# Christina-hshi/SH-assembly

Hardware: AMD Instinct MI355X
Metric: k-mers counted/sec (whole node), CQF build, C.elegans-like k=47 (higher is better)
Workload: dtype u64

## Files before the change

### sh-assembly_amd/csrc/cqf_kernels.hip

```cpp
#include "shk_device.h"

#define SHK_EMPTY 0xFFFFFFFFu
#define SHK_SUM_STRIDE 8
#define SHK_CNT_NOVER 4
#define SHK_CNT_ISLOTS 5
#define SHK_NCOUNTERS 6
#define SHK_SPILL_LENS SHK_REGION
#define SHK_SPILL_STRIDE 768
#define SHK_NC_CAP 128
#define SHK_SPILL_PACK_MAX (SHK_SPILL_STRIDE - SHK_SPILL_LENS)
#define SHK_RSCAN_TILE 4096

struct ShkMergeArgs {
  const uint8_t *tabA;
  uint8_t *tabB;
  const uint64_t *finA;
  uint64_t *finB;
  const uint32_t *words;
  const uint64_t *region_base;
  uint32_t region_cap;
  uint64_t nslots, xnslots, nblocks;
  uint64_t q_lo;
  uint32_t hb;
  uint32_t chunk_lo, chunk_hi;
  int want_hist;
  int denoise;
  uint32_t *summary;
  unsigned long long *counters;
  uint32_t *err;
  unsigned long long *dbg;
  uint32_t ablate;
  uint8_t *spill;
  const uint8_t *orec;
  uint32_t *over_list;
  unsigned long long *n_over;
  const uint32_t *list;
  uint16_t *newchunks;
  unsigned long long *chist;
  uint32_t split;
  uint32_t *isum;
  uint8_t *ilens;
  const uint64_t *prot_list;
  uint32_t nprot;
  uint32_t r0;
  uint32_t rstride;
  int counted;
};

__device__ __forceinline__ unsigned shk_img_slot_off(unsigned p) {
  return (p >> 6) * SHK_BLOCK_BYTES + SHK_OFF_SLOTS + (p & 63);
}

__device__ __forceinline__ unsigned shk_img_dec(const uint8_t *img, unsigned pos, unsigned run_end, unsigned *rem_out,
                                                uint64_t *count) {
  unsigned rem = img[shk_img_slot_off(pos)];
  *rem_out = rem;
  if (pos == run_end) { *count = 1; return 1; }
  unsigned digit = img[shk_img_slot_off(pos + 1)];
  if (digit > rem) { *count = 1; return 1; }
  unsigned n = 1;
  uint64_t cnt = 0;
  if (digit == 0) { n++; digit = img[shk_img_slot_off(pos + n)]; }
  while ((digit & 0x80) && pos + n < run_end) { cnt = cnt * 128 + (digit & 0x7f); n++; digit = img[shk_img_slot_off(pos + n)]; }
  cnt = cnt * 128 + (digit & 0x7f);
  *count = cnt + 1;
  return n + 1;
}

__device__ __forceinline__ ShkMP shk_block_exscan_mp(ShkMP v, ShkMP *total, long long *sa, long long *sb) {
  const unsigned lane = shk_lane(), wave = shk_wave(), nw = blockDim.x / SHK_WAVE;
  ShkMP incl = v;
  for (int d = 1; d < SHK_WAVE; d <<= 1) {
    ShkMP y;
    y.a = __shfl_up(incl.a, d);
    y.b = __shfl_up(incl.b, d);
    if (lane >= (unsigned)d) incl = shk_mp_compose(y, incl);
  }
  if (lane == SHK_WAVE - 1) { sa[wave] = incl.a; sb[wave] = incl.b; }
  __syncthreads();
  if (threadIdx.x == 0) {
    ShkMP run; run.a = 0; run.b = SHK_NEG_INF;
    for (unsigned w = 0; w < nw; w++) {
      ShkMP cur; cur.a = sa[w]; cur.b = sb[w];
      sa[w] = run.a; sb[w] = run.b;
      run = shk_mp_compose(run, cur);
    }
    sa[SHK_MAX_WAVES] = run.a; sb[SHK_MAX_WAVES] = run.b;
  }
  __syncthreads();
  ShkMP pre; pre.a = sa[wave]; pre.b = sb[wave];
  ShkMP prev;
  prev.a = __shfl_up(incl.a, 1);
  prev.b = __shfl_up(incl.b, 1);
  if (lane == 0) { prev.a = 0; prev.b = SHK_NEG_INF; }
  ShkMP res = shk_mp_compose(pre, prev);
  total->a = sa[SHK_MAX_WAVES];
  total->b = sb[SHK_MAX_WAVES];
  __syncthreads();
  return res;
}

__device__ __forceinline__ unsigned shk_enc_len_fast(unsigned rem, uint64_t total) {
  if (total <= 1) return (unsigned)total;
  if (total <= 128) return 2u + ((unsigned)(total - 1) > rem ? 1u : 0u);
  return shk_enc_len(rem, total);
}
__device__ __forceinline__ unsigned shk_img_dec_fast(const uint8_t *img, unsigned pos, unsigned run_end, unsigned *rem_out,
                                                     uint64_t *count) {
  const unsigned rem = img[shk_img_slot_off(pos)];
  *rem_out = rem;
  if (pos == run_end) { *count = 1; return 1; }
  const unsigned d = img[shk_img_slot_off(pos + 1)];
  if (d > rem) { *count = 1; return 1; }
  if (d != 0 && d < 0x80) { *count = (uint64_t)d + 1; return 2; }
  return shk_img_dec(img, pos, run_end, rem_out, count);
}

__device__ __forceinline__ unsigned shk_flat_dec(const uint8_t *s, unsigned pos, unsigned run_end, unsigned *rem_out, uint64_t *count) {
  unsigned rem = s[pos];
  *rem_out = rem;
  if (pos == run_end) { *count = 1; return 1; }
  unsigned digit = s[pos + 1];
  if (digit > rem) { *count = 1; return 1; }
  unsigned n = 1;
  uint64_t cnt = 0;
  if (digit == 0) { n++; digit = s[pos + n]; }
  while ((digit & 0x80) && pos + n < run_end) { cnt = cnt * 128 + (digit & 0x7f); n++; digit = s[pos + n]; }
  cnt = cnt * 128 + (digit & 0x7f);
  *count = cnt + 1;
  return n + 1;
}
__device__ __forceinline__ unsigned shk_flat_dec_fast(const uint8_t *s, unsigned pos, unsigned run_end, unsigned *rem_out, uint64_t *count) {
  const unsigned rem = s[pos];
  *rem_out = rem;
  if (pos == run_end) { *count = 1; return 1; }
  const unsigned d = s[pos + 1];
  if (d > rem) { *count = 1; return 1; }
  if (d != 0 && d < 0x80) { *count = (uint64_t)d + 1; return 2; }
  return shk_flat_dec(s, pos, run_end, rem_out, count);
}

template <int IMGB>
__device__ __forceinline__ void shk_store_image(const ShkMergeArgs &A, uint32_t r, uint32_t nregions, const uint8_t *nimg,
                                                unsigned tid, uint32_t nown, uint64_t b0, uint64_t q0, uint32_t out_lo,
                                                uint32_t out_hi, bool new_any, long long fout_rel) {
  if (r == nregions - 1) {
    const long long fend = fout_rel + (long long)q0;
    for (uint64_t b = A.nslots / 64 + tid; b < A.nblocks; b += SHK_WAVE) {
      long long o = fend - (long long)(64 * b);
      A.tabB[b * SHK_BLOCK_BYTES] = (uint8_t)(o < 0 ? 0 : (o > 255 ? 255 : o));
    }
  }

  uint8_t *tb = A.tabB + b0 * SHK_BLOCK_BYTES;
  uint32_t vblk = nown;
  if (new_any && out_lo == 0 && (nown * SHK_BLOCK_BYTES) % 4 == 0) {
    vblk = 0;
    const uint32_t *src = reinterpret_cast<const uint32_t *>(nimg);
    uint32_t *dst = reinterpret_cast<uint32_t *>(tb);
    for (uint32_t i = tid; i < nown * SHK_BLOCK_BYTES / 4; i += SHK_WAVE) dst[i] = src[i];
  }
  for (uint32_t i = tid; i < vblk * 9; i += SHK_WAVE) {
    const uint32_t blk = i / 9, byte = i % 9;
    tb[blk * SHK_BLOCK_BYTES + byte] = nimg[blk * SHK_BLOCK_BYTES + byte];
  }
  if (out_hi > out_lo) {
    const uint32_t va = vblk * 64, vb = nown * 64;
    for (uint32_t p = out_lo + tid; p < out_hi; p += SHK_WAVE)
      if (p < va || p >= vb || vblk == nown) tb[shk_img_slot_off(p)] = nimg[shk_img_slot_off(p)];
    const uint32_t m0 = out_lo >> 3, m1 = (out_hi - 1) >> 3;
    for (uint32_t m = m0 + tid; m <= m1; m += SHK_WAVE) {
      const uint32_t bo = (m >> 3) * SHK_BLOCK_BYTES + SHK_OFF_RUN + (m & 7);
      const uint8_t v = nimg[bo];
      if (vblk < nown && (m >> 3) >= vblk && (m >> 3) < nown) continue;
      if (m == m0 || m == m1) {
        if (v) {
          uint8_t *addr = tb + bo;
          uintptr_t ai = reinterpret_cast<uintptr_t>(addr);
          uint32_t *w = reinterpret_cast<uint32_t *>(ai & ~(uintptr_t)3);
          atomicOr(w, (uint32_t)v << ((ai & 3) << 3));
        }
      } else {
        tb[bo] = v;
      }
    }
  }
}

#define SHK_STAGE_PER_LANE 32
#define SHK_STAGE_STRIDE 36

#define SHK_STAMP(i) do { if (A.dbg && (blockIdx.x & 63) == 0 && threadIdx.x == 0) { unsigned long long t_ = __builtin_amdgcn_s_memtime(); atomicAdd(&A.dbg[i], t_ - t_prev); t_prev = t_; } } while (0)

template <int MODE, int IMGB, bool FUSED = false, bool OLDREC = false>
__global__ void __launch_bounds__(SHK_MERGE_GROUP) k_region_merge(ShkMergeArgs A) {
  static_assert(!FUSED || MODE == 3, "the one-pass deNoise point is a spill-mode pass");
  static_assert(!OLDREC || MODE == 0 || MODE == 3, "the write pass reads the table");
  constexpr bool WRITE = MODE == 1;
  constexpr bool STAGE = WRITE || MODE == 3;
  constexpr unsigned IMG_BLOCKS = IMGB, IMG_SLOTS = IMGB * 64, IMG_BYTES = IMGB * SHK_BLOCK_BYTES;
  static_assert(IMGB <= SHK_WAVE, "one lane per image block in the rank/select step");
  __shared__ __attribute__((aligned(16))) uint32_t hkey[SHK_HCAP];
  __shared__ __attribute__((aligned(16))) uint32_t hcnt[SHK_HCAP];
  __shared__ uint32_t s_added_b;
  __shared__ __attribute__((aligned(16))) uint16_t qcnt[SHK_REGION];
  uint32_t *qcntw = reinterpret_cast<uint32_t *>(qcnt);
  __shared__ uint16_t qoff[SHK_REGION + 2];
  __shared__ uint16_t nidx[SHK_HCAP];
  __shared__ __attribute__((aligned(8))) uint16_t orend[SHK_REGION];
  __shared__ uint16_t rstart[SHK_REGION];
  __shared__ __attribute__((aligned(16))) uint8_t oimg[IMG_BYTES + 16];
  __shared__ __attribute__((aligned(16))) uint8_t nimg[IMG_BYTES + 16];
  __shared__ __attribute__((aligned(16))) uint8_t opk[SHK_SPILL_PACK_MAX + 16];
  __shared__ __attribute__((aligned(16))) uint8_t stage[SHK_MERGE_THREADS * SHK_STAGE_STRIDE];
  __shared__ uint64_t oocc[SHK_REGION_BLOCKS];
  __shared__ uint64_t orunw[IMG_BLOCKS];
  __shared__ uint32_t oorank[SHK_REGION_BLOCKS + 1];
  __shared__ uint32_t orrank[IMG_BLOCKS + 1];
  __shared__ uint32_t s_fail, s_added, s_nlist;
  uint32_t *hidle = reinterpret_cast<uint32_t *>(orend);

  unsigned long long t_prev = A.dbg ? __builtin_amdgcn_s_memtime() : 0;
  const unsigned tid = threadIdx.x;
  const unsigned ngrp = blockDim.x;
  constexpr unsigned nthr = SHK_MERGE_THREADS;
  const uint32_t r = A.list ? A.list[blockIdx.x] : (blockIdx.x + A.r0) * A.rstride;
  const uint32_t nregions = (uint32_t)((A.nslots + SHK_REGION - 1) / SHK_REGION);
  const uint64_t q0 = (uint64_t)r * SHK_REGION;
  const uint32_t nq = (uint32_t)((A.nslots - q0) < SHK_REGION ? (A.nslots - q0) : SHK_REGION);
  const uint32_t nown = (nq + 63) / 64;
  const uint64_t b0 = q0 / 64;

  const uint64_t fa0 = A.finA[r], fa1 = A.finA[r + 1];
  const uint64_t olo_abs = fa0 > q0 ? fa0 : q0;
  const bool old_any = fa1 > olo_abs;
  const uint32_t olo = (uint32_t)(olo_abs - q0);
  const uint32_t ohi = old_any ? (uint32_t)((fa1 - q0) > 0xFFFFFFF ? 0xFFFFFFF : (fa1 - q0)) : olo;
  uint32_t nblk_old = old_any ? (ohi + 63) / 64 : 0;
  if (nblk_old < nown) nblk_old = nown;
  if (tid == 0) { s_fail = 0; s_added = 0; s_nlist = 0; s_added_b = 0; }
  uint16_t *slist = reinterpret_cast<uint16_t *>(stage);
  bool fatal = false;
  if (!OLDREC && (nblk_old > IMG_BLOCKS || ohi > IMG_SLOTS)) {
    if (tid == 0) atomicOr(A.err, SHK_E_OLD_EXTENT);
    fatal = true;
    nblk_old = nown;
  }
  if (b0 + nblk_old > A.nblocks) nblk_old = (uint32_t)(A.nblocks - b0);

  if ((MODE == 0 || MODE == 3) && !old_any && !fatal && (!A.words || (A.region_cap ? A.region_base[r] == (uint64_t)r * A.region_cap : A.region_base[r] == A.region_base[r + 1]))) {
    if (tid < SHK_SUM_STRIDE) A.summary[(size_t)SHK_SUM_STRIDE * r + tid] = 0;
    if (MODE == 3 && tid < SHK_WAVE) reinterpret_cast<uint32_t *>(A.spill + (size_t)r * SHK_SPILL_STRIDE)[tid] = 0;
    if (FUSED) {
      if (tid < 2) A.isum[2 * (size_t)r + tid] = 0;
      if (tid < SHK_WAVE) reinterpret_cast<uint32_t *>(A.ilens + (size_t)r * SHK_REGION)[tid] = 0;
    }
    return;
  }

  uint32_t ol4 = 0, oex = 0;
  bool orec_bad = false;
  {
    if (OLDREC) {
      if (tid < SHK_WAVE) {
        const uint32_t *src = reinterpret_cast<const uint32_t *>(A.orec + (size_t)r * SHK_SPILL_STRIDE);
        ol4 = src[tid];
        const uint32_t mine = (ol4 & 255u) + ((ol4 >> 8) & 255u) + ((ol4 >> 16) & 255u) + (ol4 >> 24);
        const uint32_t sincl = shk_wave_incl_add(mine);
        oex = sincl - mine;
        uint32_t ototal = (uint32_t)__builtin_amdgcn_readlane((int)sincl, SHK_WAVE - 1);
        if (ototal > SHK_SPILL_PACK_MAX) { orec_bad = true; ototal = 0; ol4 = 0; }
        uint32_t *dst = reinterpret_cast<uint32_t *>(opk);
        for (uint32_t i = tid; i < (ototal + 3) / 4; i += SHK_WAVE) dst[i] = src[SHK_SPILL_LENS / 4 + i];
      }
    } else {
    const uint32_t nbytes = nblk_old * SHK_BLOCK_BYTES;
    const uint32_t *src = reinterpret_cast<const uint32_t *>(A.tabA + b0 * SHK_BLOCK_BYTES);
    uint32_t *dst = reinterpret_cast<uint32_t *>(oimg);
    if (!(A.ablate & 64)) for (uint32_t i = tid; i < (nbytes + 3) / 4; i += ngrp) dst[i] = src[i];
    }
    {
      const uint4 e4 = make_uint4(SHK_EMPTY, SHK_EMPTY, SHK_EMPTY, SHK_EMPTY), z4 = make_uint4(0, 0, 0, 0);
      for (uint32_t i = tid; i < SHK_HCAP / 4; i += ngrp) reinterpret_cast<uint4 *>(hkey)[i] = e4;
      for (uint32_t i = tid; i < SHK_HCAP / 4; i += ngrp) reinterpret_cast<uint4 *>(hcnt)[i] = z4;
      for (uint32_t i = tid; i < SHK_REGION / 8; i += ngrp) reinterpret_cast<uint4 *>(qcnt)[i] = z4;
    }
    if (tid < 2 * SHK_WAVE) hidle[tid] = 0;
    if (WRITE) {
      uint32_t *z = reinterpret_cast<uint32_t *>(nimg);
      for (uint32_t i = tid; i < (IMG_BYTES + 16) / 4; i += ngrp) z[i] = 0;
    }
  }
  __syncthreads();

  SHK_STAMP(0);
  uint32_t my_added = 0, my_added_b = 0;
  if (A.words && !fatal && !(A.ablate & 1)) {
    const uint64_t kb = A.region_cap ? (uint64_t)r * A.region_cap : A.region_base[r], ke = A.region_cap ? A.region_base[r] : A.region_base[r + 1];
    const unsigned lane = shk_lane();
    const bool wh = A.want_hist != 0;
    bool corrupt = false, hfull = false;
    const uint32_t nw = (uint32_t)(ke - kb);
    if (FUSED && ((ke - kb) >= 32768 || A.counted) && tid == 0) atomicOr(A.err, SHK_E_FUSED);
    const uint32_t *wp = A.words + kb;
    for (uint32_t i0 = 0; i0 < nw; i0 += 4 * ngrp) {
      uint32_t wv[4];
#pragma unroll
      for (int u = 0; u < 4; u++) {
        const uint32_t i = i0 + (uint32_t)u * ngrp + tid;
        wv[u] = i < nw ? wp[i] : ~0u;
      }
      uint32_t h[4], want[4], chk[4], wgt[4];
      bool pend[4], bef[4];
#pragma unroll
      for (int u = 0; u < 4; u++) {
        const uint32_t w = wv[u];
        const bool in = i0 + (uint32_t)u * ngrp + tid < nw;
        const uint32_t chunk = w & (SHK_MAX_CHUNKS - 1);
        const uint32_t tag = (w >> SHK_CHUNK_BITS) & 0xFFFFu;
        const bool inr = in && (A.counted || (chunk >= A.chunk_lo && chunk <= A.chunk_hi));
        corrupt |= inr && (tag >> 8) >= nq;
        pend[u] = inr && (tag >> 8) < nq;
        want[u] = tag << SHK_CHUNK_BITS;
        chk[u] = chunk;
        wgt[u] = A.counted ? chunk + 1u : 1u;
        bef[u] = FUSED && chunk <= A.split;
        h[u] = (__umul24(tag, 40503u) & 0xFFFFu) >> (16 - SHK_HCAP_LOG2);
        my_added += (pend[u] && !bef[u]) ? wgt[u] : 0u;
        if (FUSED) my_added_b += (pend[u] && bef[u]) ? wgt[u] : 0u;
      }
      if (A.ablate & 256) continue;
      uint32_t guard = 0;
      while (__ballot(pend[0] || pend[1] || pend[2] || pend[3])) {
#pragma unroll
        for (int u = 0; u < 4; u++) {
          if (!__ballot(pend[u])) continue;
          const uint32_t prev = atomicCAS(pend[u] ? &hkey[h[u]] : &hidle[lane], pend[u] ? SHK_EMPTY : 0xFFFFFFFEu, want[u] | (SHK_MAX_CHUNKS - 1));
          const bool ins = pend[u] && prev == SHK_EMPTY;
          const uint32_t now = ins ? want[u] : prev;
          const bool match = pend[u] && (now >> SHK_CHUNK_BITS) == (want[u] >> SHK_CHUNK_BITS);
          const unsigned long long mi = __ballot(ins);
          if (mi) {
            const unsigned first = (unsigned)(__ffsll((long long)mi) - 1);
            uint32_t base = 0;
            if (lane == first) base = atomicAdd(&s_nlist, (uint32_t)__popcll(mi));
            base = (uint32_t)__builtin_amdgcn_readlane((int)base, (int)first);
            if (ins) slist[base + (uint32_t)__popcll(mi & ((1ULL << lane) - 1))] = (uint16_t)h[u];
          }
          if (wh) atomicMin(match ? &hkey[h[u]] : &hidle[lane], match ? (want[u] | chk[u]) : 0xFFFFFFFFu);
          atomicAdd(match ? &hcnt[h[u]] : &hidle[lane], match ? ((FUSED && !bef[u]) ? wgt[u] << 16 : wgt[u]) : 0u);
          pend[u] = pend[u] && !match;
          h[u] = pend[u] ? ((h[u] + 1) & (SHK_HCAP - 1)) : h[u];
        }
        if (A.ablate & 512) break;
        if (++guard > SHK_HCAP) { hfull = pend[0] || pend[1] || pend[2] || pend[3]; break; }
      }
    }
    if (__ballot(corrupt) && corrupt) atomicOr(A.err, SHK_E_CORRUPT);
    if (__ballot(hfull) && hfull) atomicOr(&s_fail, SHK_E_HASH_FULL);
  }
  if (my_added) atomicAdd(&s_added, my_added);
  if (FUSED && my_added_b) atomicAdd(&s_added_b, my_added_b);
  __syncthreads();
  SHK_STAMP(1);
  if (tid >= (OLDREC ? 1 : 2) * nthr) return;
  const bool helper = ngrp > nthr && tid >= nthr;
  if (!OLDREC && (helper || ngrp == nthr)) {
    const unsigned ln = tid & (SHK_WAVE - 1);
    {
      uint64_t ow = 0;
      if (ln < nown) ow = shk_ld64(oimg + ln * SHK_BLOCK_BYTES + SHK_OFF_OCC);
      if (ln < SHK_REGION_BLOCKS) oocc[ln] = ow;
      const uint32_t pc = (uint32_t)__popcll(ow);
      const uint32_t inc = shk_wave_incl_add(pc);
      if (ln < SHK_REGION_BLOCKS) oorank[ln] = inc - pc;
      if (ln == SHK_REGION_BLOCKS - 1) oorank[SHK_REGION_BLOCKS] = inc;
      uint64_t rw = 0;
      if (old_any && !fatal && ln < nblk_old) {
        rw = shk_ld64(oimg + ln * SHK_BLOCK_BYTES + SHK_OFF_RUN);
        const uint32_t s0 = ln * 64;
        if (s0 + 64 <= olo || s0 >= ohi) rw = 0;
        else {
          if (olo > s0) rw &= ~((1ULL << (olo - s0)) - 1);
          if (ohi < s0 + 64) rw &= ((1ULL << (ohi - s0)) - 1);
        }
      }
      const uint32_t rc = (uint32_t)__popcll(rw);
      const uint32_t rinc = shk_wave_incl_add(rc);
      if (ln < IMG_BLOCKS) { orrank[ln] = rinc - rc; orunw[ln] = rw; }
      if (ln == SHK_WAVE - 1) orrank[IMG_BLOCKS] = rinc;
    }
    shk_wave_sync();
    const uint32_t nruns = orrank[IMG_BLOCKS];
    if (nruns != oorank[SHK_REGION_BLOCKS] || nruns > SHK_REGION) {
      if (ln == 0) { atomicOr(A.err, SHK_E_CORRUPT); atomicOr(&s_fail, SHK_E_CORRUPT); }
    } else if (!fatal) {
      for (uint32_t j = ln; j < nruns; j += SHK_WAVE) {
        uint32_t lo = 0, hi = IMG_BLOCKS;
        while (hi - lo > 1) {
          const uint32_t mid = (lo + hi) >> 1;
          if (orrank[mid] <= j) lo = mid; else hi = mid;
        }
        orend[j] = (uint16_t)(lo * 64 + shk_select64(orunw[lo], j - orrank[lo]));
      }
    }
    if (helper) { __syncthreads(); return; }
    shk_wave_sync();
  }
  my_added = tid == 0 ? s_added : 0;
  my_added_b = (FUSED && tid == 0) ? s_added_b : 0;
  SHK_STAMP(2);
  const uint32_t nlist = (A.ablate & 16) ? 0 : s_nlist;
  for (uint32_t i = tid; i < nlist; i += nthr) { const uint32_t q = hkey[slist[i]] >> (SHK_CHUNK_BITS + 8); atomicAdd(&qcntw[q >> 1], 1u << (16 * (q & 1))); }
  shk_wave_sync();
  constexpr uint32_t per = SHK_REGION / nthr;
  const uint32_t qa = tid * per;
  {
    uint32_t sacc = 0;
#pragma unroll
    for (uint32_t j = 0; j < per; j++) sacc += qcnt[qa + j];
    uint32_t ex = shk_wave_incl_add(sacc) - sacc;
#pragma unroll
    for (uint32_t j = 0; j < per; j++) { qoff[qa + j] = (uint16_t)ex; ex += qcnt[qa + j]; }
    if (tid == nthr - 1) qoff[SHK_REGION] = (uint16_t)ex;
  }
  shk_wave_sync();
  for (uint32_t i = tid; i < nlist; i += nthr) {
    const uint32_t h = slist[i];
    const uint32_t q = hkey[h] >> (SHK_CHUNK_BITS + 8);
    const uint32_t pos = qoff[q] + (((atomicSub(&qcntw[q >> 1], 1u << (16 * (q & 1))) >> (16 * (q & 1))) & 0xFFFFu) - 1);
    nidx[pos] = (uint16_t)h;
  }
  shk_wave_sync();
  for (uint32_t j = 0; j < per; j++) {
    const uint32_t q = qa + j;
    const uint32_t a = qoff[q], b = qoff[q + 1];
    for (uint32_t i = a + 1; i < b; i++) {
      const uint16_t x = nidx[i];
      const uint32_t rx = (hkey[x] >> SHK_CHUNK_BITS) & 0xff;
      uint32_t k2 = i;
      while (k2 > a && ((hkey[nidx[k2 - 1]] >> SHK_CHUNK_BITS) & 0xff) > rx) { nidx[k2] = nidx[k2 - 1]; k2--; }
      nidx[k2] = x;
    }
  }
  if (OLDREC) shk_wave_sync();
  else __syncthreads();
  if (s_fail & SHK_E_CORRUPT) fatal = true;
  if (OLDREC && orec_bad) { fatal = true; if (tid == 0) atomicOr(A.err, SHK_E_CORRUPT); }

  SHK_STAMP(3);
  uint32_t my_new = 0, my_removed = 0;
  ShkMPw mine; mine.a = 0; mine.b = SHK_NEG_INF_W;
  ShkMPw mine_i; mine_i.a = 0; mine_i.b = SHK_NEG_INF_W;
  uint32_t l4i = 0;
  bool big_i = false;
  uint32_t st_used = 0;
  bool st_over = false;
  uint8_t *mystage = stage + tid * SHK_STAGE_STRIDE;
  if (qa < nq && !fatal && !(A.ablate & 2)) {
    static_assert(!OLDREC || per == 4, "a lane's length bytes are one dword of the record");
    const uint64_t ow = OLDREC ? 0 : oocc[qa >> 6];
    uint32_t occ4 = (uint32_t)(ow >> (qa & 63)) & ((1u << per) - 1);
    uint32_t jr = OLDREC ? 0 : oorank[qa >> 6] + (uint32_t)__popcll(ow & ((1ULL << (qa & 63)) - 1));
    uint32_t oprev = OLDREC ? 0 : (jr ? (uint32_t)orend[jr - 1] + 1 : olo);
    uint32_t oq = 0, opos = 0, oend = 0, orem = 0, on = 0;
    uint64_t ocnt = 0;
    bool ohas = false;
    auto old_decode = [&]() {
      on = OLDREC ? shk_flat_dec_fast(opk, opos, oend, &orem, &ocnt) : shk_img_dec_fast(oimg, opos, oend, &orem, &ocnt);
    };
    auto old_open_run = [&]() {
      const uint32_t j = (uint32_t)__ffs((int)occ4) - 1;
      oq = qa + j; occ4 &= occ4 - 1;
      if (OLDREC) oend = opos + ((ol4 >> (8 * j)) & 255u) - 1;
      else { oend = orend[jr]; opos = oprev > oq ? oprev : oq; }
      old_decode();
    };
    auto old_next = [&]() {
      opos += on;
      if (opos <= oend) old_decode();
      else if (occ4) {
        if (!OLDREC) { jr++; oprev = oend + 1; }
        old_open_run();
      } else ohas = false;
    };
    if (OLDREC) {
      occ4 = ((ol4 & 0xFFu) ? 1u : 0u) | ((ol4 & 0xFF00u) ? 2u : 0u) | ((ol4 & 0xFF0000u) ? 4u : 0u) | ((ol4 >> 24) ? 8u : 0u);
      opos = oex;
    }
    if (occ4) { old_open_run(); ohas = true; }
    uint32_t ni = qoff[qa];
    const uint32_t ne = qoff[qa + per];
    uint32_t nh = 0, nkey = 0;
    constexpr uint32_t NONE = 0xFFFFFFu;
    uint32_t ncomp = NONE;
    if (ni < ne) { nh = nidx[ni]; nkey = hkey[nh]; ncomp = nkey >> SHK_CHUNK_BITS; }
    uint32_t curq = 0xFFFFFFFFu, len = 0, ilen = 0;
    while (ohas || ni < ne) {
      const uint32_t ocomp = ohas ? ((oq << 8) | orem) : NONE;
      const uint32_t comp = ocomp < ncomp ? ocomp : ncomp;
      const bool take_old = ocomp == comp, take_new = ncomp == comp;
      const uint32_t eq = comp >> 8, rem = comp & 0xff;
      if (eq != curq) {
        if (len) {
          qcnt[curq] = (uint16_t)len;
          ShkMPw m; m.a = (int)len; m.b = (int)(curq + len);
          mine = shk_mpw_compose(mine, m);
        }
        if (FUSED && ilen) {
          l4i |= (ilen > 255u ? 255u : ilen) << (8 * (curq - qa)); big_i |= ilen > 255u;
          ShkMPw m; m.a = (int)ilen; m.b = (int)(curq + ilen);
          mine_i = shk_mpw_compose(mine_i, m);
        }
        curq = eq; len = 0; ilen = 0;
      }
      uint64_t total = 0;
      bool is_new = false;
      uint32_t nhx = 0;
      if (FUSED) {
        uint64_t cb = take_old ? ocnt : 0, ca = 0;
        if (take_old) old_next();
        if (take_new) {
          { const uint32_t c2 = hcnt[nh]; cb += c2 & 0xFFFFu; ca = c2 >> 16; }
          if (A.newchunks && !take_old) hcnt[nh] = 0x80000000u;
          ni++;
          ncomp = NONE;
          if (ni < ne) { nh = nidx[ni]; nkey = hkey[nh]; ncomp = nkey >> SHK_CHUNK_BITS; }
        }
        if (cb) ilen += shk_enc_len_fast(rem, cb);
        bool prot = false;
        if (cb == 1) {
          if (A.prot_list) {
            const uint64_t gq = q0 + eq;
            uint32_t lo2 = 0, hi2 = A.nprot;
            while (lo2 < hi2) { const uint32_t mid = (lo2 + hi2) >> 1; if (A.prot_list[mid] < gq) lo2 = mid + 1; else hi2 = mid; }
            prot = lo2 < A.nprot && A.prot_list[lo2] == gq;
          }
          if (!prot) my_removed++;
        }
        const uint64_t kept = cb >= 2 ? cb : (prot ? 1 : 0);
        total = kept + ca;
        if (total == 0) continue;
        if (kept == 0) my_new++;
      } else {
      if (take_old) {
        total = ocnt;
        if (!OLDREC && A.denoise) {
          const uint32_t tb = (opos >> 6) * SHK_BLOCK_BYTES + SHK_OFF_TRAV + ((opos & 63) >> 3);
          const bool prot = (oimg[tb] >> (opos & 7)) & 1;
          if (ocnt < 2 && !prot) { my_removed++; total = 0; is_new = true; }
        }
        old_next();
      } else is_new = true;
      if (take_new) {
        total += hcnt[nh];
        nhx = nh;
        ni++;
        ncomp = NONE;
        if (ni < ne) { nh = nidx[ni]; nkey = hkey[nh]; ncomp = nkey >> SHK_CHUNK_BITS; }
      } else is_new = false;
      if (total == 0) continue;
      }
      if (!FUSED && is_new) {
        my_new++;
        if (MODE != 1 && A.want_hist && A.newchunks) hcnt[nhx] |= 0x80000000u;
      }
      const unsigned el = shk_enc_len_fast(rem, total);
      if (STAGE) {
        if (!st_over && st_used + el <= SHK_STAGE_PER_LANE) {
          if (total <= 128) {
            mystage[st_used] = (uint8_t)rem;
            if (total > 1) {
              const unsigned cdig = (unsigned)(total - 1);
              unsigned o = 1;
              if (cdig > rem) mystage[st_used + o++] = 0;
              mystage[st_used + o] = (uint8_t)cdig;
            }
          } else {
            uint8_t enc[12];
            const unsigned n = shk_enc_write(enc, rem, total);
            for (unsigned i = 0; i < n; i++) mystage[st_used + i] = enc[i];
          }
          st_used += el;
        } else st_over = true;
      }
      len += el;
    }
    if (len) {
      qcnt[curq] = (uint16_t)len;
      ShkMPw m; m.a = (int)len; m.b = (int)(curq + len);
      mine = shk_mpw_compose(mine, m);
    }
    if (FUSED && ilen) {
      l4i |= (ilen > 255u ? 255u : ilen) << (8 * (curq - qa)); big_i |= ilen > 255u;
      ShkMPw m; m.a = (int)ilen; m.b = (int)(curq + ilen);
      mine_i = shk_mpw_compose(mine_i, m);
    }
  }
  SHK_STAMP(4);
  if (FUSED) {
    const ShkMPw inc_i = shk_mpw_wave_scan(mine_i);
    reinterpret_cast<uint32_t *>(A.ilens + (size_t)r * SHK_REGION)[tid] = l4i;
    if (__ballot(big_i) && tid == 0) atomicOr(A.err, SHK_E_FUSED);
    if (tid == SHK_WAVE - 1) {
      A.isum[2 * (size_t)r] = fatal ? 0 : (uint32_t)inc_i.a;
      A.isum[2 * (size_t)r + 1] = (!fatal && inc_i.b > 0) ? (uint32_t)inc_i.b : 0;
      if (inc_i.a > 0xFFFF) atomicOr(A.err, SHK_E_FUSED);
    }
  }
  const ShkMPw incl = shk_mpw_wave_scan(mine);
  ShkMP tot, pre;
  tot.a = __builtin_amdgcn_readlane(incl.a, SHK_WAVE - 1);
  { const int tb = __builtin_amdgcn_readlane(incl.b, SHK_WAVE - 1); tot.b = tb > 0 ? tb : SHK_NEG_INF; }
  pre.a = 0; pre.b = SHK_NEG_INF;
  if (MODE == 1) {
    pre.a = __shfl_up(incl.a, 1);
    { const int pb = __shfl_up(incl.b, 1); pre.b = pb > 0 ? pb : SHK_NEG_INF; }
    if (tid == 0) { pre.a = 0; pre.b = SHK_NEG_INF; }
  }

  if (MODE != 1) {
    const uint32_t t_added = shk_wave_incl_add(my_added), t_new = shk_wave_incl_add(my_new),
                   t_removed = shk_wave_incl_add(my_removed), t_before = FUSED ? shk_wave_incl_add(my_added_b) : 0;
    if (tid == SHK_WAVE - 1) {
      uint32_t *sm = A.summary + (size_t)SHK_SUM_STRIDE * r;
      sm[0] = fatal ? 0 : (uint32_t)tot.a;
      sm[1] = (!fatal && tot.b > 0) ? (uint32_t)tot.b : 0;
      sm[2] = t_new; sm[3] = t_added; sm[4] = t_removed; sm[5] = t_before;
      if (!(A.want_hist && A.newchunks && !fatal)) sm[7] = 0;
      if (tot.a > 0xFFFF) atomicOr(A.err, SHK_E_RUN_TOO_LONG);
      if (s_fail) atomicOr(A.err, s_fail);
    }
  }
  SHK_STAMP(5);
  if (MODE != 1 && A.want_hist && A.newchunks && !fatal) {
    uint16_t *nc = A.newchunks + (size_t)r * SHK_NC_CAP;
    uint32_t base = 0;
    for (uint32_t i0 = 0; i0 < nlist; i0 += SHK_WAVE) {
      const uint32_t h = i0 + tid < nlist ? nidx[i0 + tid] : 0;
      const bool f = i0 + tid < nlist && (hcnt[h] >> 31);
      const unsigned long long m = __ballot(f);
      if (f) {
        const uint32_t at = base + (uint32_t)__popcll(m & ((1ULL << tid) - 1));
        const uint32_t ch = hkey[h] & (SHK_MAX_CHUNKS - 1);
        if (at < SHK_NC_CAP) nc[at] = (uint16_t)ch;
        else atomicAdd(&A.chist[ch], 1ULL);
      }
      base += (uint32_t)__popcll(m);
    }
    if (tid == 0) A.summary[(size_t)SHK_SUM_STRIDE * r + 7] = base < SHK_NC_CAP ? base : SHK_NC_CAP;
  }
  if (MODE == 3) {
    uint8_t *sp = A.spill + (size_t)r * SHK_SPILL_STRIDE;
    uint32_t l4 = 0;
    bool big = st_over;
#pragma unroll
    for (uint32_t j = 0; j < per; j++) {
      const uint32_t len = qcnt[qa + j];
      if (len > 255) big = true;
      l4 |= (len & 255u) << (8 * j);
    }
    reinterpret_cast<uint32_t *>(sp)[tid] = l4;
    const uint32_t sincl = shk_wave_incl_add(st_used);
    const uint32_t stot = (uint32_t)__builtin_amdgcn_readlane((int)sincl, SHK_WAVE - 1);
    const bool over = !fatal && (__ballot(big) != 0 || stot > SHK_SPILL_PACK_MAX);
    if (tid == 0) {
      A.summary[(size_t)SHK_SUM_STRIDE * r + 6] = over ? 1 : 0;
      if (over) A.over_list[atomicAdd(A.n_over, 1ULL)] = r;
      if (over && FUSED) atomicOr(A.err, SHK_E_FUSED);
    }
    if (!over) {
      const uint32_t ex = sincl - st_used;
      for (uint32_t i = 0; i < st_used; i++) sp[SHK_SPILL_LENS + ex + i] = mystage[i];
    }
    return;
  }
  if (MODE == 0 || (A.ablate & 128)) return;

  const long long fin_rel = (long long)A.finB[r] - (long long)q0;
  const long long fout_rel = (long long)A.finB[r + 1] - (long long)q0;
  if (fatal) return;
  const uint32_t out_lo = fin_rel > 0 ? (uint32_t)fin_rel : 0;
  const bool new_any = tot.a > 0;
  const uint32_t out_hi = new_any ? (uint32_t)fout_rel : out_lo;
  if (new_any && (fout_rel > IMG_SLOTS || fout_rel < 0)) {
    if (tid == 0) atomicOr(A.err, SHK_E_NEW_EXTENT);
    return;
  }
  uint32_t *nimg32 = reinterpret_cast<uint32_t *>(nimg);
  {
    long long f = shk_mp_apply(pre, fin_rel);
    uint32_t so = 0;
    for (uint32_t j = 0; j < per; j++) {
      const uint32_t q = qa + j;
      if (q < nq && (q & 63) == 0) {
        long long o = f - (long long)q;
        nimg[(q >> 6) * SHK_BLOCK_BYTES] = (uint8_t)(o < 0 ? 0 : (o > 255 ? 255 : o));
      }
      const uint32_t len = qcnt[q];
      if (len) {
        const long long stt = f > (long long)q ? f : (long long)q;
        rstart[q] = (uint16_t)stt;
        f = stt + len;
        if (!st_over) {
          const uint32_t wp = (uint32_t)stt;
          for (uint32_t i = 0; i < len; i++) nimg[shk_img_slot_off(wp + i)] = mystage[so + i];
          so += len;
          const uint32_t last = wp + len - 1;
          const uint32_t bo = (last >> 6) * SHK_BLOCK_BYTES + SHK_OFF_RUN + ((last & 63) >> 3);
          atomicOr(&nimg32[bo >> 2], 1u << (((bo & 3) << 3) + (last & 7)));
          const uint32_t oo = (q >> 6) * SHK_BLOCK_BYTES + SHK_OFF_OCC + ((q & 63) >> 3);
          atomicOr(&nimg32[oo >> 2], 1u << (((oo & 3) << 3) + (q & 7)));
        }
      }
    }
// ... 574 lines not shown
```

Measured before the change: 37.48 billion.

## Compact pending probes into a queue and build the slot list by scanning the hash table

The hash-insert loop now packs each record's tag, chunk and pending flag into one word. After one probe per record, it compacts the still-pending records so each lane drains a short queue, instead of re-ballotting over all four unrolled slots each round. The per-insert ballot and shared atomicAdd that appended to the slot list are removed. The list of used slots is instead rebuilt after the insert phase by scanning the hash keys with a wave prefix sum, which also gives a deterministic order. This lowers LDS atomic and ballot traffic in the hot loop, at the cost of a full hash-table scan and a changed table-full detection rule.

```diff
diff --git a/sh-assembly_amd/csrc/cqf_kernels.hip b/sh-assembly_amd/csrc/cqf_kernels.hip
--- a/sh-assembly_amd/csrc/cqf_kernels.hip
+++ b/sh-assembly_amd/csrc/cqf_kernels.hip
@@ -187,6 +187,8 @@
   }
 }
 
+__device__ __forceinline__ uint32_t shk_fold_home(uint32_t tag) { return (__umul24(tag, 40503u) & 0xFFFFu) >> (16 - SHK_HCAP_LOG2); }
+
 #define SHK_STAGE_PER_LANE 32
 #define SHK_STAGE_STRIDE 36
 
@@ -217,7 +219,7 @@
   __shared__ uint64_t orunw[IMG_BLOCKS];
   __shared__ uint32_t oorank[SHK_REGION_BLOCKS + 1];
   __shared__ uint32_t orrank[IMG_BLOCKS + 1];
-  __shared__ uint32_t s_fail, s_added, s_nlist;
+  __shared__ uint32_t s_fail, s_added;
   uint32_t *hidle = reinterpret_cast<uint32_t *>(orend);
 
   unsigned long long t_prev = A.dbg ? __builtin_amdgcn_s_memtime() : 0;
@@ -238,7 +240,7 @@
   const uint32_t ohi = old_any ? (uint32_t)((fa1 - q0) > 0xFFFFFFF ? 0xFFFFFFF : (fa1 - q0)) : olo;
   uint32_t nblk_old = old_any ? (ohi + 63) / 64 : 0;
   if (nblk_old < nown) nblk_old = nown;
-  if (tid == 0) { s_fail = 0; s_added = 0; s_nlist = 0; s_added_b = 0; }
+  if (tid == 0) { s_fail = 0; s_added = 0; s_added_b = 0; }
   uint16_t *slist = reinterpret_cast<uint16_t *>(stage);
   bool fatal = false;
   if (!OLDREC && (nblk_old > IMG_BLOCKS || ohi > IMG_SLOTS)) {
@@ -303,6 +305,20 @@
     const uint32_t nw = (uint32_t)(ke - kb);
     if (FUSED && ((ke - kb) >= 32768 || A.counted) && tid == 0) atomicOr(A.err, SHK_E_FUSED);
     const uint32_t *wp = A.words + kb;
+    static_assert(16 + SHK_CHUNK_BITS < 31, "a record's tag and chunk leave bit 31 free");
+    constexpr uint32_t QPEND = 0x80000000u, QTAG = 0xFFFFu << SHK_CHUNK_BITS;
+    auto probe = [&](uint32_t qw, uint32_t hh) -> bool {
+      const bool p = (qw & QPEND) != 0;
+      const uint32_t want = qw & QTAG, chk = qw & (SHK_MAX_CHUNKS - 1);
+      const uint32_t wgt = A.counted ? chk + 1u : 1u;
+      const bool bef = FUSED && chk <= A.split;
+      const uint32_t prev = atomicCAS(p ? &hkey[hh] : &hidle[lane], p ? SHK_EMPTY : 0xFFFFFFFEu, want | (SHK_MAX_CHUNKS - 1));
+      const uint32_t now = (p && prev == SHK_EMPTY) ? want : prev;
+      const bool match = p && (now >> SHK_CHUNK_BITS) == (want >> SHK_CHUNK_BITS);
+      if (wh) atomicMin(match ? &hkey[hh] : &hidle[lane], match ? (want | chk) : 0xFFFFFFFFu);
+      atomicAdd(match ? &hcnt[hh] : &hidle[lane], match ? ((FUSED && !bef) ? wgt << 16 : wgt) : 0u);
+      return match;
+    };
     for (uint32_t i0 = 0; i0 < nw; i0 += 4 * ngrp) {
       uint32_t wv[4];
 #pragma unroll
@@ -310,8 +326,7 @@
         const uint32_t i = i0 + (uint32_t)u * ngrp + tid;
         wv[u] = i < nw ? wp[i] : ~0u;
       }
-      uint32_t h[4], want[4], chk[4], wgt[4];
-      bool pend[4], bef[4];
+      uint32_t q[4], qh[4];
 #pragma unroll
       for (int u = 0; u < 4; u++) {
         const uint32_t w = wv[u];
@@ -320,40 +335,53 @@
         const uint32_t tag = (w >> SHK_CHUNK_BITS) & 0xFFFFu;
         const bool inr = in && (A.counted || (chunk >= A.chunk_lo && chunk <= A.chunk_hi));
         corrupt |= inr && (tag >> 8) >= nq;
-        pend[u] = inr && (tag >> 8) < nq;
-        want[u] = tag << SHK_CHUNK_BITS;
-        chk[u] = chunk;
-        wgt[u] = A.counted ? chunk + 1u : 1u;
-        bef[u] = FUSED && chunk <= A.split;
-        h[u] = (__umul24(tag, 40503u) & 0xFFFFu) >> (16 - SHK_HCAP_LOG2);
-        my_added += (pend[u] && !bef[u]) ? wgt[u] : 0u;
-        if (FUSED) my_added_b += (pend[u] && bef[u]) ? wgt[u] : 0u;
+        const bool pend = inr && (tag >> 8) < nq;
+        const uint32_t wgt = A.counted ? chunk + 1u : 1u;
+        const bool bef = FUSED && chunk <= A.split;
+        q[u] = (w & (QTAG | (SHK_MAX_CHUNKS - 1))) | (pend ? QPEND : 0u);
+        qh[u] = shk_fold_home(tag);
+        my_added += (pend && !bef) ? wgt : 0u;
+        if (FUSED) my_added_b += (pend && bef) ? wgt : 0u;
       }
       if (A.ablate & 256) continue;
-      uint32_t guard = 0;
-      while (__ballot(pend[0] || pend[1] || pend[2] || pend[3])) {
-#pragma unroll
-        for (int u = 0; u < 4; u++) {
-          if (!__ballot(pend[u])) continue;
-          const uint32_t prev = atomicCAS(pend[u] ? &hkey[h[u]] : &hidle[lane], pend[u] ? SHK_EMPTY : 0xFFFFFFFEu, want[u] | (SHK_MAX_CHUNKS - 1));
-          const bool ins = pend[u] && prev == SHK_EMPTY;
-          const uint32_t now = ins ? want[u] : prev;
-          const bool match = pend[u] && (now >> SHK_CHUNK_BITS) == (want[u] >> SHK_CHUNK_BITS);
-          const unsigned long long mi = __ballot(ins);
-          if (mi) {
-            const unsigned first = (unsigned)(__ffsll((long long)mi) - 1);
-            uint32_t base = 0;
-            if (lane == first) base = atomicAdd(&s_nlist, (uint32_t)__popcll(mi));
-            base = (uint32_t)__builtin_amdgcn_readlane((int)base, (int)first);
-            if (ins) slist[base + (uint32_t)__popcll(mi & ((1ULL << lane) - 1))] = (uint16_t)h[u];
-          }
-          if (wh) atomicMin(match ? &hkey[h[u]] : &hidle[lane], match ? (want[u] | chk[u]) : 0xFFFFFFFFu);
-          atomicAdd(match ? &hcnt[h[u]] : &hidle[lane], match ? ((FUSED && !bef[u]) ? wgt[u] << 16 : wgt[u]) : 0u);
-          pend[u] = pend[u] && !match;
-          h[u] = pend[u] ? ((h[u] + 1) & (SHK_HCAP - 1)) : h[u];
-        }
-        if (A.ablate & 512) break;
-        if (++guard > SHK_HCAP) { hfull = pend[0] || pend[1] || pend[2] || pend[3]; break; }
+#pragma unroll
+      for (int u = 0; u < 4; u++) {
+        if (!__ballot(q[u] & QPEND)) continue;
+        const bool match = probe(q[u], qh[u]);
+        q[u] = match ? 0u : q[u];
+        qh[u] = (qh[u] + 1) & (SHK_HCAP - 1);
+      }
+      if (A.ablate & 512) continue;
+      if (!__ballot((q[0] | q[1] | q[2] | q[3]) & QPEND)) continue;
+#pragma unroll
+      for (int pass = 0; pass < 3; pass++) {
+#pragma unroll
+        for (int u = 0; u < 3 - pass; u++) {
+          const bool hole = !(q[u] & QPEND);
+          qh[u] = hole ? qh[u + 1] : qh[u];
+          const uint32_t up = hole ? 0u : q[u + 1];
+          q[u] = hole ? q[u + 1] : q[u];
+          q[u + 1] = up;
+        }
+      }
+      uint32_t steps = 0;
+      while (__ballot(q[0] & QPEND)) {
+        const bool p = (q[0] & QPEND) != 0;
+        const bool match = probe(q[0], qh[0]);
+        const uint32_t nh = (qh[0] + 1) & (SHK_HCAP - 1);
+        bool keep = p && !match;
+        if (++steps >= SHK_HCAP - 1) {
+          const bool full = keep && nh == shk_fold_home((q[0] & QTAG) >> SHK_CHUNK_BITS);
+          hfull |= full;
+          keep = keep && !full;
+        }
+        qh[0] = keep ? nh : qh[1];
+        q[0] = keep ? q[0] : q[1];
+        qh[1] = keep ? qh[1] : qh[2];
+        q[1] = keep ? q[1] : q[2];
+        qh[2] = keep ? qh[2] : qh[3];
+        q[2] = keep ? q[2] : q[3];
+        q[3] = keep ? q[3] : 0u;
       }
     }
     if (__ballot(corrupt) && corrupt) atomicOr(A.err, SHK_E_CORRUPT);
@@ -410,7 +438,28 @@
   my_added = tid == 0 ? s_added : 0;
   my_added_b = (FUSED && tid == 0) ? s_added_b : 0;
   SHK_STAMP(2);
-  const uint32_t nlist = (A.ablate & 16) ? 0 : s_nlist;
+  uint32_t nlist;
+  {
+    constexpr uint32_t EPL = SHK_HCAP / nthr;
+    static_assert(EPL % 4 == 0 && EPL <= 32, "whole 16-byte reads; a lane's entries in one mask");
+    uint32_t used = 0;
+#pragma unroll
+    for (uint32_t j = 0; j < EPL; j += 4) {
+      const uint4 k4 = reinterpret_cast<const uint4 *>(hkey)[(tid * EPL + j) / 4];
+      used |= (uint32_t)(k4.x != SHK_EMPTY) << j | (uint32_t)(k4.y != SHK_EMPTY) << (j + 1) | (uint32_t)(k4.z != SHK_EMPTY) << (j + 2) | (uint32_t)(k4.w != SHK_EMPTY) << (j + 3);
+    }
+    const uint32_t mine = (uint32_t)__popc(used);
+    const uint32_t incl = shk_wave_incl_add(mine);
+    uint32_t pos = incl - mine;
+#pragma unroll
+    for (uint32_t j = 0; j < EPL; j++) {
+      if ((used >> j) & 1u) slist[pos] = (uint16_t)(tid * EPL + j);
+      pos += (used >> j) & 1u;
+    }
+    nlist = (uint32_t)__builtin_amdgcn_readlane((int)incl, SHK_WAVE - 1);
+    if (A.ablate & 16) nlist = 0;
+  }
+  shk_wave_sync();
   for (uint32_t i = tid; i < nlist; i += nthr) { const uint32_t q = hkey[slist[i]] >> (SHK_CHUNK_BITS + 8); atomicAdd(&qcntw[q >> 1], 1u << (16 * (q & 1))); }
   shk_wave_sync();
   constexpr uint32_t per = SHK_REGION / nthr;
```

New measurement: 39.25 billion (median of 6 runs). +4.7%, better.
